# retinal-information-processing-lab/gaussian_processes

Hardware: AMD Instinct MI355X
Metric: GP fits/sec (kernel+chol+solve+grad loglik) at N=8192 d=256 (higher is better)
Workload: dtype f64; 1 GPU; N=8192 d=256 single cell f64, one M-step closure evaluation with 6 gradients (BASELINE configs[2], headline); N=8192, d=256, parallelism=independent units over 1 GPU(s), one process per GPU, no data-path collective

## Files before the change

gaussian_processes_amd/_lib.py:

```python
from __future__ import annotations

import ctypes
import os

from .build import lib_path

vp, i32, i64, f64 = ctypes.c_void_p, ctypes.c_int, ctypes.c_int64, ctypes.c_double
pd = ctypes.POINTER(ctypes.c_double)

_SIGS = {
    "gpfit_version": (i32, []),
    "gpfit_last_error": (ctypes.c_char_p, []),
    "gpfit_dgemm": (i32, [vp, i32, i32, i32, i32, i32, f64, vp, i64, vp, i64, f64, vp, i64, i32, i32, i32]),
    "gpfit_dgemm_ex": (i32, [vp, i32, i32, i32, i32, i32, f64, vp, i64, vp, i64, f64, vp, i64, i32, i32, i32, i32, i32]),
    "gpfit_ctx_create": (i32, [i32, i64, i64, i64, ctypes.POINTER(vp)]),
    "gpfit_ctx_destroy": (None, [vp]),
    "gpfit_check_limits": (i32, [pd, pd, pd]),
    "gpfit_localker_mask": (i32, [pd, i32, i32, vp, ctypes.POINTER(i64)]),
    "gpfit_localker": (i32, [vp, vp, pd, i32, i32, vp, i64, vp, vp]),
    "gpfit_acosker": (i32, [vp, vp, f64, vp, i64, i64, vp, i64, i64, i64, vp, i64, vp, vp, i64, vp]),
    "gpfit_acosker_pullback": (i32, [vp, vp, f64, vp, i64, i64, vp, i64, i64, i64, vp, i64, vp, i64, vp, vp, i64, pd]),
    "gpfit_acosker_diag": (i32, [vp, vp, f64, vp, i64, i64, i64, vp, i64, vp, vp, vp]),
    "gpfit_fit_eval": (i32, [vp, vp, pd, pd, pd, i32, i32, vp, i64, i64, vp, vp, vp, i64, f64, f64, i32, pd,
                             vp, vp, vp]),
    "gpfit_potrf": (i32, [vp, vp, vp, i64, i64, vp, i64, vp, i64, pd, ctypes.POINTER(i32)]),
    "gpfit_potrf_append": (i32, [vp, vp, vp, i64, vp, i64, i64, vp, pd, ctypes.POINTER(i32)]),
    "gpfit_estep": (i32, [vp, vp, vp, i64, i64, vp, vp, vp, f64, vp, vp, i64]),
    "gpfit_estep_projected": (i32, [vp, vp, vp, i64, vp, i64, vp, i64, i64, i64, vp, vp, vp, f64, vp, vp, i64, vp, vp,
                                    vp]),
    "gpfit_fparam_eval": (i32, [vp, vp, vp, vp, vp, i64, f64, i32, f64, vp, pd]),
    "gpfit_fparam_lbfgs": (i32, [vp, vp, vp, vp, vp, i64, f64, i32, f64, i32, i32, f64, f64, f64, vp, pd]),
    "gpfit_fparam_lbfgs_host": (i32, [vp, vp, vp, i64, f64, i32, f64, i32, i32, f64, f64, f64, vp, pd]),
    "gpfit_set_profile": (i32, [vp, i32]),
    "gpfit_get_profile": (i32, [vp, pd]),
    "gpfit_get_phases": (i32, [vp, pd]),
    "gpfit_last_enqueue_ms": (f64, [vp]),
    "gpfit_fit_eval_f32": (i32, [vp, vp, pd, pd, pd, i32, i32, vp, i64, i64, vp, vp, vp, i64, f64, f64, i32, pd,
                                 vp, vp, vp]),
    "gpfit_fit_eval_finish": (i32, [vp, pd]),
    "gpfit_fit_eval_batch": (i32, [vp, i32, vp, pd, pd, pd, i32, i32, vp, i64, i64, vp, vp, vp, i64, pd, pd, i32, pd,
                                   ctypes.POINTER(i32)]),
    "gpfit_fit_eval_batch_f32": (i32, [vp, i32, vp, pd, pd, pd, i32, i32, vp, i64, i64, vp, vp, vp, i64, pd, pd, i32, pd,
                                       ctypes.POINTER(i32)]),
    "gpfit_fit_eval_projected": (i32, [vp, vp, pd, pd, pd, i32, i32, vp, i64, i64, vp, vp, i64, i64, vp, vp, i64, f64, f64, pd]),
    "gpfit_fit_eval_sparse": (i32, [vp, vp, pd, pd, pd, i32, i32, vp, i64, i64, vp, i64, i64, vp, vp, i64, i64, vp, vp, i64,
                                    f64, f64, pd]),
    "gpfit_grad_pullback": (i32, [vp, vp, pd, i32, i32, vp, i64, i64, vp, i64, vp, pd]),
    "gpfit_nd_utility": (i32, [vp, vp, vp, i64, vp, i32, vp]),
    "gpfit_probe_mfma_f64": (i32, [vp, vp, i32, i32]),
    "gpfit_probe_stream_copy": (i32, [vp, vp, vp, i64]),
}

_lib = None


class GpfitError(RuntimeError):
    pass


def exported_symbols():
    return sorted(_SIGS)


def load():
    global _lib
    if _lib is not None:
        return _lib
    path = lib_path()
    if not os.path.exists(path):
        raise GpfitError(
            f"{path} not found: build it with `python -m gaussian_processes_amd.build` "
            "(there is no CPU fallback for the GP fit path)")
    lib = ctypes.CDLL(path)
    for name, (res, args) in _SIGS.items():
        fn = getattr(lib, name)
        fn.restype = res
        fn.argtypes = args
    _lib = lib
    return lib


def last_error() -> str:
    return load().gpfit_last_error().decode(errors="replace")
# ... 11 lines not shown
```

gaussian_processes_amd/csrc/common.h:

```cpp
#pragma once
#include <hip/hip_runtime.h>
#include <stdint.h>
#include <stdio.h>
#include <string>

namespace gpfit {

constexpr double PI32 = 3.1415927410125732;

constexpr int TILE = 128;
constexpr int TRMV_ROWS = 128;
constexpr int KTILE = 16;

void set_error(const std::string& msg);

#define GP_HIP(expr)                                                                     \
  do {                                                                                   \
    hipError_t _e = (expr);                                                              \
    if (_e != hipSuccess) {                                                              \
      gpfit::set_error(std::string(#expr) + ": " + hipGetErrorString(_e));               \
      return -100;                                                                       \
    }                                                                                    \
  } while (0)

// ... 21 lines not shown
  int batch;
  int64_t sA, sB, sC;
  int split_k;
  int tile;
  int reverse;
  int workspace;
  void* sk_ws;
  int tile_limit;
  int half_occ;
  const int* sched;
  int sched_blocks;
  int epi;
  R* aux;
  double* sumsq;
  int nptr;
  const R* Ap[GEMM_MAXB];
  const R* Bp[GEMM_MAXB];
  R* Cp[GEMM_MAXB];
  R* auxp[GEMM_MAXB];
  double* sumsqp[GEMM_MAXB];
};
using GemmArgs = GemmArgsT<double>;

constexpr size_t SK_WS_BYTES = (size_t)2 * 512 * TILE * TILE * sizeof(double);

template <typename R> constexpr int ktile_of() { return 128 / (int)sizeof(R); }

template <typename R> int launch_gemm(const GemmArgsT<R>& a, hipStream_t s);
template <typename R> int gemm_pick_tile(const GemmArgsT<R>& a);
template <typename R> int launch_gemm_streamk(const GemmArgsT<R>& a, hipStream_t s);
template <typename R> int launch_gemm_plain(const GemmArgsT<R>& a, hipStream_t s);
template <typename R> bool gemm_pair_ok(const GemmArgsT<R>& a, const GemmArgsT<R>& b);
template <typename R> int launch_gemm_pair(const GemmArgsT<R>& a, const GemmArgsT<R>& b, hipStream_t s);
template <typename R> int launch_gemm_xcd(const GemmArgsT<R>& a, hipStream_t s);
template <typename R> bool gemm_epilogue_ok(const GemmArgsT<R>& a);
template <typename R> bool gemm_streamk_applies(const GemmArgsT<R>& a);
template <typename R> bool gemm_streamk_carries(const GemmArgsT<R>& a);
template <typename R> int gemm_sumsq_entries(const GemmArgsT<R>& a);
template <typename R> bool gemm_xcd_applies(const GemmArgsT<R>& a);

template <typename R>
struct GramArgsT {
  const R* XCt;
  const R* Xt;
  const R* q1;
  const R* q2;
  R* Kout;
  R* Cos;
  int64_t ld1, ld2, ldk;
  int64_t ldcos;
  int np1, np2, nv1, nv2, Kd;
  double s0sq;
  int lower;
  int pad_identity;
  int mirror;
};
using GramArgs = GramArgsT<double>;
template <typename R> int launch_gram(const GramArgsT<R>& a, hipStream_t s);

}
```

gaussian_processes_amd/csrc/fit.hip:

```cpp
#include "context.h"
#include "gpfit_mi355x.h"

#include <algorithm>
#include <chrono>
#include <cmath>
#include <cstdlib>
#include <cstring>
#include <limits>

namespace gpfit {

static thread_local gpfit_ctx* g_prof = nullptr;
static thread_local void* g_main_sk_ws = nullptr;

static const int* walks() {
  static int w[7] = {3, 2, 1, 9, 9, 2, 2};
  static bool init = false;
  if (!init) {
    init = true;
    if (const char* e = getenv("GPFIT_WALKS")) {
      int v[7];
      if (sscanf(e, "%d,%d,%d,%d,%d,%d,%d", &v[0], &v[1], &v[2], &v[3], &v[4], &v[5], &v[6]) == 7)
        for (int i = 0; i < 7; ++i) w[i] = v[i];
    }
// ... 81 lines not shown
                              int b_tri, int reverse = 0, int ws = 0, void* sk_ws = nullptr) {
  GemmArgsT<R> g{};
  g.A = A; g.B = B; g.C = C;
  g.lda = lda; g.ldb = ldb; g.ldc = ldc;
  g.M = M; g.N = N; g.K = K;
  g.alpha = alpha; g.beta = beta;
  g.a_kmajor = a_kmajor; g.b_kmajor = b_kmajor;
  g.out_lower = out_lower; g.a_tri = a_tri; g.b_tri = b_tri;
  g.batch = 1; g.split_k = 1; g.reverse = reverse; g.workspace = ws; g.sk_ws = sk_ws ? sk_ws : g_main_sk_ws;
  return g;
}

static int g_eval_count = 0;
static int gemm_log_eval() {
  static const int v = getenv("GPFIT_GEMM_LOG") ? atoi(getenv("GPFIT_GEMM_LOG")) : -1;
  return v;
}

template <typename R>
static int run_gemm(hipStream_t s, const GemmArgsT<R>& g) {
  if (gemm_log_eval() >= 0 && g_eval_count == gemm_log_eval())
    fprintf(stderr, "[gpfit gemm] M %d N %d K %d atri %d btri %d lower %d nb %d tile %d ak %d bk %d epi %d flops %.6e\n", g.M, g.N, g.K,
            g.a_tri, g.b_tri, g.out_lower, g.nptr > 0 ? g.nptr : 1, gemm_pick_tile(g), g.a_kmajor, g.b_kmajor, g.epi, gemm_flops(g));
  ProfScope ps(s, g_prof ? gemm_flops(g) : 0.0, (g_prof && gemm_pick_tile(g) != TILE) ? 3 : 0);
  return launch_gemm(g, s);
}

template <typename R>
static int gemm(hipStream_t s, int a_kmajor, int b_kmajor, int M, int N, int K, double alpha, const R* A,
                int64_t lda, const R* B, int64_t ldb, double beta, R* C, int64_t ldc, int out_lower, int a_tri,
                int b_tri, int reverse = 0, int ws = 0, void* sk_ws = nullptr) {
  return run_gemm(s, gemm_args<R>(a_kmajor, b_kmajor, M, N, K, alpha, A, lda, B, ldb, beta, C, ldc, out_lower, a_tri, b_tri,
                                  reverse, ws, sk_ws));
}

template <typename R>
static int gemm_splitk(hipStream_t s, int a_kmajor, int b_kmajor, int M, int N, int K, double alpha, const R* A, int64_t lda,
                       const R* B, int64_t ldb, R* C, int64_t ldc, int splits, R* partial, int64_t partial_elems) {
  static const bool off = getenv("GPFIT_NO_SPLITK") != nullptr;
  splits = (int)std::min<int64_t>(splits, partial_elems / std::max<int64_t>(1, (int64_t)M * ldc));
  if (splits <= 1 || off || partial == nullptr)
    return gemm<R>(s, a_kmajor, b_kmajor, M, N, K, alpha, A, lda, B, ldb, 0.0, C, ldc, 0, 0, 0);
  GemmArgsT<R> g = gemm_args<R>(a_kmajor, b_kmajor, M, N, K, alpha, A, lda, B, ldb, 0.0, partial, ldc, 0, 0, 0);
  g.split_k = splits;
  g.sC = (int64_t)M * ldc;
  g.tile = TILE;
  GP_TRY(run_gemm(s, g));
  return launch_reduce_slices(partial, (int64_t)M * ldc, splits, C, (int64_t)M * ldc, s);
}
static int splitk_for(int M, int N, int K) {
  const long tiles = (long)((M + TILE - 1) / TILE) * ((N + TILE - 1) / TILE);
  if (tiles >= 384) return 1;
  long sp = (768 + tiles - 1) / tiles;
  sp = std::min<long>(sp, std::max(1, K / 256));
  return (int)std::max<long>(1, sp);
}

static int fused_epilogues() {
  static const int v = getenv("GPFIT_FUSED_EPI") ? atoi(getenv("GPFIT_FUSED_EPI")) : 7;
  return v;
}


template <typename R>
static int gemm_list(hipStream_t s, int cnt, const R* const* Ap, const R* const* Bp, R* const* Cp, int a_kmajor,
                     int b_kmajor, int M, int N, int K, double alpha, int64_t lda, int64_t ldb, double beta, int64_t ldc,
// ... 580 lines not shown
  const int kt = np / TILE, n1 = ((kt + 1) / 2) * TILE, n2 = np - n1;
  int ent = 0;
  auto asks = [&](int M, int Nn, int K, int lower, int a_tri, int b_tri, int walk) {
    GemmArgsT<R> g1 = gemm_args<R>(0, 1, M, Nn, K, 1.0, a[0].Li, ld, a[0].LV, ld, 0.0, a[0].T, ld, lower, a_tri, b_tri, walk, 0, cs[0]->sk_ws[0]);
    g1.epi = 2; g1.sumsq = cs[0]->frob_part;
    return ((fused_epilogues() & 2) && gemm_pick_tile(g1) == TILE) ? gemm_sumsq_entries(g1) : 0;
  };
  const bool any_fused = asks(n1, n1, n1, 1, 1, 1, walks()[3]) > 0 || asks(n2, n2, n2, 1, 1, 1, walks()[3]) > 0 ||
                         asks(n2, n1, n2, 0, 1, 0, walks()[2]) > 0;
  auto diag_blocks = [&](int cb, const int* rb, int nblk) -> int {
    const int tb = nblk / TILE;
    int e = asks(nblk, nblk, nblk, 1, 1, 1, walks()[3]);
    const bool ask = e > 0;
    if (!ask) e = tb * (tb + 1) / 2;
    int m = 0;
    for (int i = 0; i < cnt; ++i)
      for (int j = 0; j < cb; ++j, ++m) {
        const int64_t o = (int64_t)rb[j] * ld + rb[j];
        Ap[m] = a[i].Li + o; Bp[m] = a[i].LV + o; Tp[m] = a[i].T + o; Sp[m] = cs[i]->frob_part + ent + j * e;
      }
    bool normed = false;
    GP_TRY(gemm_list<R>(s, m, Ap, Bp, Tp, 0, 1, nblk, nblk, nblk, 1.0, ld, ld, 0.0, ld, 1, 1, 1, walks()[3], 0, cs[0]->sk_ws[0],
                        ask ? 2 : 0, nullptr, Sp, &normed));
    if (normed != ask) {
      set_error("post_join: the tile-norm epilogue of a diagonal block of T was announced but not carried");
      return -100;
    }
    if (!normed && any_fused)
      for (int q = 0; q < m; ++q) GP_TRY(launch_frob_tiles<R>(Tp[q], ld, nblk, nblk, 1, Sp[q], s));
    ent += cb * e;
    return 0;
  };
  const int r_both[2] = {0, n1};
  if (n2 == n1 && 2 * cnt <= GEMM_MAXB) GP_TRY(diag_blocks(2, r_both, n1));
  else {
    GP_TRY(diag_blocks(1, r_both, n1));
    GP_TRY(diag_blocks(1, r_both + 1, n2));
  }
  {
    const int64_t o21 = (int64_t)n1 * ld;
    for (int i = 0; i < cnt; ++i) {
      GP_HIP(hipMemcpy2DAsync(a[i].Z + o21, (size_t)ld * sizeof(R), a[i].LV + o21, (size_t)ld * sizeof(R), (size_t)n1 * sizeof(R),
                              (size_t)n2, hipMemcpyDeviceToDevice, s));
      Ap[i] = a[i].L + o21; Bp[i] = a[i].T; Cp[i] = a[i].Z + o21;
    }
    GP_TRY(gemm_list<R>(s, cnt, Ap, Bp, Cp, 0, 1, n2, n1, n1, -1.0, ld, ld, 1.0, ld, 0, 0, 1, walks()[1], 0, cs[0]->sk_ws[0]));
    int e = asks(n2, n1, n2, 0, 1, 0, walks()[2]);
    const bool ask = e > 0;
    if (!ask) e = (n2 / TILE) * (n1 / TILE);
    for (int i = 0; i < cnt; ++i) {
      Ap[i] = a[i].Li + o21 + n1; Bp[i] = a[i].Z + o21; Tp[i] = a[i].T + o21; Sp[i] = cs[i]->frob_part + ent;
    }
    bool normed = false;
    GP_TRY(gemm_list<R>(s, cnt, Ap, Bp, Tp, 0, 1, n2, n1, n2, 1.0, ld, ld, 0.0, ld, 0, 1, 0, walks()[2], 0, cs[0]->sk_ws[0],
                        ask ? 2 : 0, nullptr, Sp, &normed));
    if (normed != ask) {
      set_error("post_join: the tile-norm epilogue of T21 was announced but not carried");
      return -100;
    }
    if (!normed && any_fused)
      for (int i = 0; i < cnt; ++i) GP_TRY(launch_frob_tiles<R>(Tp[i], ld, n2, n1, 0, Sp[i], s));
    ent += e;
  }
  for (int i = 0; i < cnt; ++i) {
    if (any_fused) GP_TRY(launch_frob_finish(cs[i]->frob_part, ent, cs[i]->scal + 5, s));
    else GP_TRY(launch_frob_lower(a[i].T, ld, np, cs[i]->scal + 5, cs[i]->frob_part, s));
  }
  return 0;
}

template <typename R, typename PhaseFn>
static int post_join_list(int cnt, gpfit_ctx* const* cs, const PostJoin<R>* a, const Theta* th, int n, int np, const int* d,
                          const int* dp, int n_rows, int n_cols, int want_grad, bool blocks, hipStream_t s, PhaseFn&& phase) {
  const int64_t ld = np;
  const R* Ap[GEMM_MAXB];
  const R* Bp[GEMM_MAXB];
  R* Cp[GEMM_MAXB];
  double* Sp[GEMM_MAXB];
  if (cnt <= 0 || cnt > GEMM_MAXB) return cnt == 0 ? 0 : -3;
// ... 766 lines not shown
```

gaussian_processes_amd/csrc/gemm.hip:

```cpp
#include "gemm_core.h"

#include <algorithm>
#include <cstdlib>
#include <mutex>
#include <set>
#include <utility>

namespace gpfit {

template <typename R, bool A_KMAJOR, bool B_KMAJOR, bool EDGE, int T, int NS>
__device__ __forceinline__ bool gemm_tile_compute(const GemmArgsT<R>& p, int tiles_n, int ntiles, R* smem,
                                                  typename Real<R>::acc_t (&acc)[T / 32][T / 32], int& ti, int& tj,
                                                  int& row0, int& col0, R*& C) {
  constexpr int KT = Real<R>::KT;

  const int bid = (p.reverse & 1) ? (ntiles - 1 - (int)blockIdx.x) : (int)blockIdx.x;
  if (p.sched != nullptr) {
    const int e = p.sched[blockIdx.x];
    if (e < 0) return false;
    ti = e >> 16;
    tj = e & 0xffff;
  } else if (p.out_lower && (p.reverse & 2) && T == TILE) {
    const int nt = tiles_n;
    int j = (int)((2.0 * nt + 1.0 - sqrt((2.0 * nt + 1.0) * (2.0 * nt + 1.0) - 8.0 * (double)bid)) * 0.5);
    while (j > 0 && (long)j * nt - (long)j * (j - 1) / 2 > bid) --j;
    while ((long)(j + 1) * nt - (long)(j + 1) * j / 2 <= bid) ++j;
    tj = j;
    ti = j + (bid - (j * nt - j * (j - 1) / 2));
  } else if (p.out_lower) {
    lower_tile(bid, TILE / T, ti, tj);
  } else if (p.reverse & 2) {
    const int tiles_m = ntiles / tiles_n;
    tj = bid / tiles_m;
    ti = bid % tiles_m;
  } else {
    ti = bid / tiles_n;
    tj = bid % tiles_n;
  }
  row0 = ti * T;
  col0 = tj * T;
  const int b = blockIdx.y, z = blockIdx.z;
  const R* A;
  const R* B;
  if (p.nptr > 0) {
    A = p.Ap[b];
    B = p.Bp[b];
    C = p.Cp[b];
  } else {
    A = p.A + (int64_t)b * p.sA;
    B = p.B + (int64_t)b * p.sB;
    C = p.C + (int64_t)b * p.sC;
  }

  int kbeg = 0, kend = p.K;
  if (p.a_tri == 1) kend = min(kend, row0 + T);
  if (p.a_tri == 2) kbeg = max(kbeg, row0);
  if (p.b_tri == 1) kbeg = max(kbeg, col0);
  if (p.b_tri == 2) kend = min(kend, col0 + T);
  if (p.split_k > 1) {
    const int steps = max(0, kend - kbeg) / KT;
    const int per = (steps + p.split_k - 1) / p.split_k;
    const int s0 = min(steps, z * per), s1 = min(steps, (z + 1) * per);
    kend = kbeg + s1 * KT;
    kbeg = kbeg + s0 * KT;
    C += (int64_t)z * p.sC;
  }

#pragma unroll
  for (int i = 0; i < T / 32; ++i)
#pragma unroll
    for (int j = 0; j < T / 32; ++j) acc[i][j] = acc_zero<R>();

  gemm_mainloop<R, A_KMAJOR, B_KMAJOR, EDGE, T, 0, NS>(A, p.lda, B, p.ldb, p.M, p.N, row0, col0, kbeg, kend, smem, acc,
                                                       (p.reverse & 4) != 0);
  return true;
}

template <typename R, bool A_KMAJOR, bool B_KMAJOR, bool EDGE, int T, int NS, int EPI = 0>
__device__ __forceinline__ void gemm_tile_body(const GemmArgsT<R>& p, int tiles_n, int ntiles, R* smem) {
  typename Real<R>::acc_t acc[T / 32][T / 32];
  int ti, tj, row0, col0;
  R* C;
  if (!gemm_tile_compute<R, A_KMAJOR, B_KMAJOR, EDGE, T, NS>(p, tiles_n, ntiles, smem, acc, ti, tj, row0, col0, C)) return;

  const R alpha = (R)p.alpha, beta = (p.split_k > 1) ? (R)0 : (R)p.beta;
  const int64_t ldc = p.ldc;
  const int M = p.M, N = p.N;
  if constexpr (EPI != 0) {
    constexpr int epi = EPI;
    R* __restrict__ D = p.nptr > 0 ? p.auxp[blockIdx.y] : p.aux;
    double* __restrict__ sumsq = p.nptr > 0 ? p.sumsqp[blockIdx.y] : p.sumsq;
    double ss = 0.0;
    for_each_acc<R, T>(acc, row0, col0, [&](int row, int col, R v) {
      if (EDGE && !(row < M && col < N)) return;
      R o = alpha * v;
      R* c = C + (int64_t)row * ldc + col;
      if (epi & 4) {
        R* dd = D + (int64_t)row * ldc + col;
        const R d0 = *dd;
        o += d0;
        *dd = o + d0;
      } else if (beta != (R)0) {
        o += beta * (*c);
      }
      if (epi & 1) {
        if (row >= col) *c = o;
        if (row > col) C[(int64_t)col * ldc + row] = o;
// ... 274 lines not shown
int launch_gemm_pair(const GemmArgsT<R>& a, const GemmArgsT<R>& b, hipStream_t s) {
  if (!gemm_pair_ok(a, b)) {
    set_error("launch_gemm_pair: the two problems cannot share a launch (ask gemm_pair_ok first)");
    return -3;
  }
  static_assert(sizeof(GemmPairT<R>) <= 4096, "kernel arguments are limited to 4 KiB");
  const int T = pair_member_tile(a);
  GemmPairT<R> q;
  int gx = 0, gy = 0;
  long total = 0;
  for (int w = 0; w < 2; ++w) {
    q.g[w] = w == 0 ? a : b;
    GemmArgsT<R>& p = q.g[w];
    p.batch = p.nptr;
    const int tm = p.M / T, tn = p.N / T;
    q.tiles_n[w] = tn;
    q.tiles[w] = p.out_lower ? lower_tile_count(p.M / TILE, TILE / T) : tm * tn;
    gx = std::max(gx, q.tiles[w]);
    gy = std::max(gy, p.batch);
    total += (long)q.tiles[w] * p.batch;
  }
  const dim3 grid(gx, gy, 2), block(GEMM_THREADS);
  static const int deep_max = getenv("GPFIT_DEEP_MAX") ? atoi(getenv("GPFIT_DEEP_MAX")) : 512;
  if (T == 32 && total <= deep_max) hipLaunchKernelGGL((gemm_pair_kernel<R, 32, 8>), grid, block, 0, s, q);
  else if (T == 32) hipLaunchKernelGGL((gemm_pair_kernel<R, 32, 2>), grid, block, 0, s, q);
  else if (total <= deep_max) hipLaunchKernelGGL((gemm_pair_kernel<R, 64, 4>), grid, block, 0, s, q);
  else hipLaunchKernelGGL((gemm_pair_kernel<R, 64, 2>), grid, block, 0, s, q);
  GP_HIP(hipGetLastError());
  return 0;
}
template int launch_gemm_pair<double>(const GemmArgsT<double>&, const GemmArgsT<double>&, hipStream_t);
template int launch_gemm_pair<float>(const GemmArgsT<float>&, const GemmArgsT<float>&, hipStream_t);

template int launch_gemm<double>(const GemmArgsT<double>&, hipStream_t);
template int launch_gemm<float>(const GemmArgsT<float>&, hipStream_t);
template int launch_gemm_plain<double>(const GemmArgsT<double>&, hipStream_t);
template int launch_gemm_plain<float>(const GemmArgsT<float>&, hipStream_t);
template int gemm_pick_tile<double>(const GemmArgsT<double>&);
template int gemm_pick_tile<float>(const GemmArgsT<float>&);

}

#ifdef GPFIT_CLOCK_STAMPS
extern "C" int gpfit_dev_gemm_clock(long long* host_out ) {
  return hipMemcpyFromSymbol(host_out, HIP_SYMBOL(gpfit::g_gemm_clock), sizeof(long long) * 2 * 4096 * 2) == hipSuccess ? 0 : -1;
}
#endif
```

gaussian_processes_amd/csrc/gemm_sched.hip:

```cpp
#include "gemm_core.h"

#include <algorithm>
#include <cstdlib>
#include <map>
#include <mutex>
#include <tuple>
#include <vector>

namespace gpfit {

namespace {
struct Plan {
  int* table = nullptr;
  int blocks = 0;
};
using Key = std::tuple<int, int, int, int, int, int, int, int>;
std::map<Key, Plan> g_plans;
std::mutex g_mutex;

struct Item {
  long weight;
  std::vector<int> tiles;
};
}
// ... 76 lines not shown
}
template bool gemm_xcd_applies<double>(const GemmArgsT<double>&);
template bool gemm_xcd_applies<float>(const GemmArgsT<float>&);

template <typename R>
int launch_gemm_xcd(const GemmArgsT<R>& a, hipStream_t s) {
  if (!gemm_xcd_applies(a)) return 1;
  int device = 0;
  GP_HIP(hipGetDevice(&device));
  Plan plan;
  {
    std::lock_guard<std::mutex> lock(g_mutex);
    const Key key{device, a.M, a.N, a.K, a.out_lower, a.a_tri, a.b_tri, (int)sizeof(R)};
    auto it = g_plans.find(key);
    if (it == g_plans.end()) {
      Plan np;
      const int rc = build(a, np);
      if (rc != 0) return rc;
      it = g_plans.emplace(key, np).first;
    }
    plan = it->second;
  }
  GemmArgsT<R> p = a;
  p.tile = TILE;
  p.sched = plan.table;
  p.sched_blocks = plan.blocks;
  p.reverse &= 4;
  return launch_gemm_plain(p, s);
}

template int launch_gemm_xcd<double>(const GemmArgsT<double>&, hipStream_t);
template int launch_gemm_xcd<float>(const GemmArgsT<float>&, hipStream_t);

}
```

gaussian_processes_amd/csrc/probe.hip:

```cpp
#include "common.h"
#include "gpfit_mi355x.h"

namespace gpfit {
typedef double v4d __attribute__((ext_vector_type(4)));

#define GP_MFMA(acc) asm volatile("v_mfma_f64_16x16x4_f64 %0, %1, %2, %0" : "+v"(acc) : "v"(a), "v"(b))
__global__ __launch_bounds__(256) void mfma_f64_probe_kernel(double* out, int iters, double seed) {
  v4d c0 = {0, 0, 0, 0}, c1 = c0, c2 = c0, c3 = c0, c4 = c0, c5 = c0, c6 = c0, c7 = c0;
  v4d c8 = c0, c9 = c0, c10 = c0, c11 = c0, c12 = c0, c13 = c0, c14 = c0, c15 = c0;
  double a = seed + threadIdx.x * 1e-3, b = seed - threadIdx.x * 1e-3;
  for (int it = 0; it < iters; ++it) {
    GP_MFMA(c0); GP_MFMA(c1); GP_MFMA(c2); GP_MFMA(c3); GP_MFMA(c4); GP_MFMA(c5); GP_MFMA(c6); GP_MFMA(c7);
    GP_MFMA(c8); GP_MFMA(c9); GP_MFMA(c10); GP_MFMA(c11); GP_MFMA(c12); GP_MFMA(c13); GP_MFMA(c14); GP_MFMA(c15);
  }
  v4d s = c0 + c1 + c2 + c3 + c4 + c5 + c6 + c7 + c8 + c9 + c10 + c11 + c12 + c13 + c14 + c15;
  out[blockIdx.x * blockDim.x + threadIdx.x] = s[0] + s[1] + s[2] + s[3];
}
#undef GP_MFMA

__global__ void stream_copy_kernel(const double2* __restrict__ in, double2* __restrict__ out, int64_t n) {
  int64_t i = (int64_t)blockIdx.x * blockDim.x + threadIdx.x;
  const int64_t stride = (int64_t)gridDim.x * blockDim.x;
  for (; i < n; i += stride) out[i] = in[i];
}
}

extern "C" {

int gpfit_probe_mfma_f64(void* stream, double* scratch , int blocks, int iters) {
  hipLaunchKernelGGL(gpfit::mfma_f64_probe_kernel, dim3(blocks), dim3(256), 0, (hipStream_t)stream, scratch,
                     iters, 1.0);
  GP_HIP(hipGetLastError());
  return 0;
}

int gpfit_probe_stream_copy(void* stream, const double* in, double* out, int64_t n_doubles) {
  hipLaunchKernelGGL(gpfit::stream_copy_kernel, dim3(2048), dim3(256), 0, (hipStream_t)stream,
                     (const double2*)in, (double2*)out, n_doubles / 2);
  GP_HIP(hipGetLastError());
  return 0;
}
}
```

include/gpfit_mi355x.h:

```cpp
#ifndef GPFIT_MI355X_H
#define GPFIT_MI355X_H

#include <stdint.h>

#ifdef __cplusplus
extern "C" {
#endif

#define GPFIT_VERSION 100

int gpfit_version(void);
const char* gpfit_last_error(void);

int gpfit_dgemm(void* stream, int a_kmajor, int b_kmajor, int M, int N, int K, double alpha,
                const double* A, int64_t lda, const double* B, int64_t ldb, double beta, double* C,
                int64_t ldc, int out_lower, int a_tri, int b_tri);
int gpfit_dgemm_ex(void* stream, int a_kmajor, int b_kmajor, int M, int N, int K, double alpha,
                   const double* A, int64_t lda, const double* B, int64_t ldb, double beta, double* C,
                   int64_t ldc, int out_lower, int a_tri, int b_tri, int walk, int tile);

typedef struct gpfit_ctx gpfit_ctx;
int gpfit_ctx_create(int device, int64_t n_max, int64_t d_max, int64_t d_full_max, gpfit_ctx** out);
void gpfit_ctx_destroy(gpfit_ctx* ctx);

// ... 64 lines not shown
                          const double* L, int64_t ldl, int64_t N, int64_t nb, const double* r, const double* m,
                          const double* f, double logA, double* m_new, double* V_new, int64_t ldv, const double* kv0,
                          double* lam_m_out, double* lam_var_out);

int gpfit_fparam_eval(gpfit_ctx* ctx, void* stream, const double* lam_m, const double* lam_var,
                      const double* r, int64_t N, double logA, int closed_form_lambda0, double lambda0_in,
                      double* f_out, double* out_host);

int gpfit_fparam_lbfgs(gpfit_ctx* ctx, void* stream, const double* lam_m, const double* lam_var,
                       const double* r, int64_t N, double logA0, int lambda0_mode, double lambda0_fixed,
                       int max_iter, int history_size, double lr, double tol_grad, double tol_change,
                       double* f_out, double* out_host);
int gpfit_fparam_lbfgs_host(const double* lam_m, const double* lam_var, const double* r, int64_t N,
                            double logA0, int lambda0_mode, double lambda0_fixed, int max_iter,
                            int history_size, double lr, double tol_grad, double tol_change, double* f_out,
                            double* out_host);

int gpfit_nd_utility(void* stream, const double* sigma2, const double* mu, int64_t nstar, const double* r,
                     int nr, double* U);

int gpfit_set_profile(gpfit_ctx* ctx, int on);
int gpfit_get_profile(gpfit_ctx* ctx, double* out16);
int gpfit_get_phases(gpfit_ctx* ctx, double* out8);
double gpfit_last_enqueue_ms(gpfit_ctx* ctx);

int gpfit_fit_eval_f32(gpfit_ctx* ctx, void* stream, const double* theta, const double* lower,
                       const double* upper, int n_rows, int n_cols, const float* X, int64_t ldx, int64_t N,
                       const float* r, const float* m, const float* V, int64_t ldv, double logA, double lambda0,
                       int want_grad, double* out_host, float* lam_m, float* lam_var, float* f);

int gpfit_probe_mfma_f64(void* stream, double* scratch, int blocks, int iters);
int gpfit_probe_stream_copy(void* stream, const double* in, double* out, int64_t n_doubles);

#ifdef __cplusplus
}
#endif
#endif
```

Measured before the change: 35.92 fits/s.

## Fuse two dependent-free block GEMMs into one multi-problem launch with tile table

Adds a grouped GEMM kernel that runs several independent problems (up to 4 shapes × 16 members) in one launch, driven by a precomputed, load-balanced tile table cached on the device. In the blocked post-join step it merges the off-diagonal update (Z21 = LV21 - L21·T) with the lower-triangular 22 block product into one launch. It reads LV through an aux pointer in the epilogue, which removes the separate 2D device copy. This is meant to cut launch count, copy traffic and tail idle time. The cost is extra code paths, a fixed tile choice with no split-k or stream-k, and a plan cache held per shape.

```diff
diff --git a/gaussian_processes_amd/_lib.py b/gaussian_processes_amd/_lib.py
--- a/gaussian_processes_amd/_lib.py
+++ b/gaussian_processes_amd/_lib.py
@@ -49,6 +49,8 @@
     "gpfit_nd_utility": (i32, [vp, vp, vp, i64, vp, i32, vp]),
     "gpfit_probe_mfma_f64": (i32, [vp, vp, i32, i32]),
     "gpfit_probe_stream_copy": (i32, [vp, vp, vp, i64]),
+    "gpfit_probe_gemm_multi": (i32, [vp, i32, i32, i32, vp, vp, vp, vp]),
+    "gpfit_gemm_multi_table": (i32, [i32, vp, i32, i32, i32, vp, i32]),
 }
 
 _lib = None
diff --git a/gaussian_processes_amd/csrc/common.h b/gaussian_processes_amd/csrc/common.h
--- a/gaussian_processes_amd/csrc/common.h
+++ b/gaussian_processes_amd/csrc/common.h
@@ -77,6 +77,14 @@
 template <typename R> int launch_gemm_plain(const GemmArgsT<R>& a, hipStream_t s);
 template <typename R> bool gemm_pair_ok(const GemmArgsT<R>& a, const GemmArgsT<R>& b);
 template <typename R> int launch_gemm_pair(const GemmArgsT<R>& a, const GemmArgsT<R>& b, hipStream_t s);
+constexpr int MULTI_MAXD = 4;
+constexpr int MULTI_MAXB = 16;
+template <typename R> bool gemm_multi_ok(int nd, const GemmArgsT<R>* g);
+template <typename R> int gemm_multi_tile(int nd, const GemmArgsT<R>* g);
+template <typename R> int launch_gemm_multi(int nd, const GemmArgsT<R>* g, hipStream_t s);
+struct MultiShape { int M, N, K, out_lower, a_tri, b_tri; };
+int gemm_multi_table(int nd, const MultiShape* sh, int members, int T, int kstep, int* out, int cap);
+int gemm_multi_plan(int nd, const MultiShape* sh, int members, int T, int kstep, const int** table, int* blocks);
 template <typename R> int launch_gemm_xcd(const GemmArgsT<R>& a, hipStream_t s);
 template <typename R> bool gemm_epilogue_ok(const GemmArgsT<R>& a);
 template <typename R> bool gemm_streamk_applies(const GemmArgsT<R>& a);
diff --git a/gaussian_processes_amd/csrc/fit.hip b/gaussian_processes_amd/csrc/fit.hip
--- a/gaussian_processes_amd/csrc/fit.hip
+++ b/gaussian_processes_amd/csrc/fit.hip
@@ -137,6 +137,33 @@
                 int b_tri, int reverse = 0, int ws = 0, void* sk_ws = nullptr) {
   return run_gemm(s, gemm_args<R>(a_kmajor, b_kmajor, M, N, K, alpha, A, lda, B, ldb, beta, C, ldc, out_lower, a_tri, b_tri,
                                   reverse, ws, sk_ws));
+}
+
+static int no_multi() {
+  static const int v = getenv("GPFIT_NO_MULTI") ? atoi(getenv("GPFIT_NO_MULTI")) : 0;
+  return v;
+}
+
+template <typename R>
+static int run_gemm_multi(hipStream_t s, int nd, const GemmArgsT<R>* g) {
+  const int T = gemm_multi_tile(nd, g);
+  double flops = 0.0;
+  const bool log = gemm_log_eval() >= 0 && g_eval_count == gemm_log_eval();
+  if (log || g_prof)
+    for (int w = 0; w < nd; ++w) {
+      GemmArgsT<R> c = g[w];
+      c.tile = T;
+      flops += gemm_flops(c);
+    }
+  if (log) {
+    fprintf(stderr, "[gpfit gemm] multi: nd %d nb %d tile %d flops %.6e :", nd, g[0].nptr, T, flops);
+    for (int w = 0; w < nd; ++w)
+      fprintf(stderr, " [M %d N %d K %d atri %d btri %d lower %d epi %d]", g[w].M, g[w].N, g[w].K, g[w].a_tri, g[w].b_tri,
+              g[w].out_lower, g[w].epi);
+    fprintf(stderr, "\n");
+  }
+  ProfScope ps(s, g_prof ? flops : 0.0, (g_prof && T != TILE) ? 3 : 0);
+  return launch_gemm_multi(nd, g, s);
 }
 
 template <typename R>
@@ -783,19 +810,49 @@
     return 0;
   };
   const int r_both[2] = {0, n1};
-  if (n2 == n1 && 2 * cnt <= GEMM_MAXB) GP_TRY(diag_blocks(2, r_both, n1));
+  const int64_t o21 = (int64_t)n1 * ld, o22 = o21 + n1;
+  GemmArgsT<R> gm[2];
+  auto pair_args = [&](int i0, int m, bool ask22) {
+    gm[0] = gemm_args<R>(0, 1, n2, n1, n1, -1.0, (const R*)nullptr, ld, (const R*)nullptr, ld, 1.0, (R*)nullptr, ld, 0, 0, 1, walks()[1], 0,
+                         cs[0]->sk_ws[0]);
+    gm[1] = gemm_args<R>(0, 1, n2, n2, n2, 1.0, (const R*)nullptr, ld, (const R*)nullptr, ld, 0.0, (R*)nullptr, ld, 1, 1, 1, walks()[3], 0,
+                         cs[0]->sk_ws[0]);
+    gm[0].reverse &= 4; gm[1].reverse &= 4;
+    gm[1].epi = ask22 ? 2 : 0;
+    for (int w = 0; w < 2; ++w) { gm[w].nptr = m; gm[w].batch = m; }
+    for (int j = 0; j < m; ++j) {
+      const PostJoin<R>& u = a[i0 + j];
+      gm[0].Ap[j] = u.L + o21; gm[0].Bp[j] = u.T; gm[0].Cp[j] = u.Z + o21; gm[0].auxp[j] = const_cast<R*>(u.LV) + o21;
+      gm[1].Ap[j] = u.Li + o22; gm[1].Bp[j] = u.LV + o22; gm[1].Cp[j] = u.T + o22;
+      gm[1].sumsqp[j] = cs[i0 + j]->frob_part + ent;
+    }
+  };
+  const bool ask22 = asks(n2, n2, n2, 1, 1, 1, walks()[3]) > 0;
+  pair_args(0, std::min(cnt, MULTI_MAXB), ask22);
+  const bool multi = !(no_multi() & 1) && n2 > 0 && gemm_multi_ok(2, gm);
+  if (multi) {
+    GP_TRY(diag_blocks(1, r_both, n1));
+    for (int i0 = 0; i0 < cnt; i0 += MULTI_MAXB) {
+      pair_args(i0, std::min(cnt - i0, MULTI_MAXB), ask22);
+      GP_TRY(run_gemm_multi<R>(s, 2, gm));
+    }
+    if (!ask22 && any_fused)
+      for (int i = 0; i < cnt; ++i) GP_TRY(launch_frob_tiles<R>(a[i].T + o22, ld, n2, n2, 1, cs[i]->frob_part + ent, s));
+    ent += (n2 / TILE) * (n2 / TILE + 1) / 2;
+  } else if (n2 == n1 && 2 * cnt <= GEMM_MAXB) GP_TRY(diag_blocks(2, r_both, n1));
   else {
     GP_TRY(diag_blocks(1, r_both, n1));
     GP_TRY(diag_blocks(1, r_both + 1, n2));
   }
   {
-    const int64_t o21 = (int64_t)n1 * ld;
-    for (int i = 0; i < cnt; ++i) {
-      GP_HIP(hipMemcpy2DAsync(a[i].Z + o21, (size_t)ld * sizeof(R), a[i].LV + o21, (size_t)ld * sizeof(R), (size_t)n1 * sizeof(R),
-                              (size_t)n2, hipMemcpyDeviceToDevice, s));
-      Ap[i] = a[i].L + o21; Bp[i] = a[i].T; Cp[i] = a[i].Z + o21;
-    }
-    GP_TRY(gemm_list<R>(s, cnt, Ap, Bp, Cp, 0, 1, n2, n1, n1, -1.0, ld, ld, 1.0, ld, 0, 0, 1, walks()[1], 0, cs[0]->sk_ws[0]));
+    if (!multi) {
+      for (int i = 0; i < cnt; ++i) {
+        GP_HIP(hipMemcpy2DAsync(a[i].Z + o21, (size_t)ld * sizeof(R), a[i].LV + o21, (size_t)ld * sizeof(R), (size_t)n1 * sizeof(R),
+                                (size_t)n2, hipMemcpyDeviceToDevice, s));
+        Ap[i] = a[i].L + o21; Bp[i] = a[i].T; Cp[i] = a[i].Z + o21;
+      }
+      GP_TRY(gemm_list<R>(s, cnt, Ap, Bp, Cp, 0, 1, n2, n1, n1, -1.0, ld, ld, 1.0, ld, 0, 0, 1, walks()[1], 0, cs[0]->sk_ws[0]));
+    }
     int e = asks(n2, n1, n2, 0, 1, 0, walks()[2]);
     const bool ask = e > 0;
     if (!ask) e = (n2 / TILE) * (n1 / TILE);
diff --git a/gaussian_processes_amd/csrc/gemm.hip b/gaussian_processes_amd/csrc/gemm.hip
--- a/gaussian_processes_amd/csrc/gemm.hip
+++ b/gaussian_processes_amd/csrc/gemm.hip
@@ -7,6 +7,17 @@
 #include <utility>
 
 namespace gpfit {
+
+template <typename R, bool A_KMAJOR, bool B_KMAJOR, bool EDGE, int T, int NS>
+__device__ __forceinline__ void gemm_tile_product(const R* A, int64_t lda, const R* B, int64_t ldb, int M, int N, int row0,
+                                                  int col0, int kbeg, int kend, R* smem,
+                                                  typename Real<R>::acc_t (&acc)[T / 32][T / 32], bool kdesc) {
+#pragma unroll
+  for (int i = 0; i < T / 32; ++i)
+#pragma unroll
+    for (int j = 0; j < T / 32; ++j) acc[i][j] = acc_zero<R>();
+  gemm_mainloop<R, A_KMAJOR, B_KMAJOR, EDGE, T, 0, NS>(A, lda, B, ldb, M, N, row0, col0, kbeg, kend, smem, acc, kdesc);
+}
 
 template <typename R, bool A_KMAJOR, bool B_KMAJOR, bool EDGE, int T, int NS>
 __device__ __forceinline__ bool gemm_tile_compute(const GemmArgsT<R>& p, int tiles_n, int ntiles, R* smem,
@@ -66,13 +77,8 @@
     C += (int64_t)z * p.sC;
   }
 
-#pragma unroll
-  for (int i = 0; i < T / 32; ++i)
-#pragma unroll
-    for (int j = 0; j < T / 32; ++j) acc[i][j] = acc_zero<R>();
-
-  gemm_mainloop<R, A_KMAJOR, B_KMAJOR, EDGE, T, 0, NS>(A, p.lda, B, p.ldb, p.M, p.N, row0, col0, kbeg, kend, smem, acc,
-                                                       (p.reverse & 4) != 0);
+  gemm_tile_product<R, A_KMAJOR, B_KMAJOR, EDGE, T, NS>(A, p.lda, B, p.ldb, p.M, p.N, row0, col0, kbeg, kend, smem, acc,
+                                                        (p.reverse & 4) != 0);
   return true;
 }
 
@@ -413,6 +419,157 @@
 template int launch_gemm_pair<double>(const GemmArgsT<double>&, const GemmArgsT<double>&, hipStream_t);
 template int launch_gemm_pair<float>(const GemmArgsT<float>&, const GemmArgsT<float>&, hipStream_t);
 
+template <typename R>
+struct GemmDescT {
+  int64_t lda, ldb, ldc;
+  int M, N, K;
+  double alpha, beta;
+  int out_lower, a_tri, b_tri, epi, tiles_n, kdesc;
+  const R* Ap[MULTI_MAXB];
+  const R* Bp[MULTI_MAXB];
+  R* Cp[MULTI_MAXB];
+  R* auxp[MULTI_MAXB];
+  double* sumsqp[MULTI_MAXB];
+};
+template <typename R>
+struct GemmMultiT {
+  GemmDescT<R> d[MULTI_MAXD];
+  const int* table;
+};
+
+template <typename R, int T, int NS>
+__device__ __forceinline__ void gemm_multi_body(const GemmMultiT<R>& q, R* smem) {
+  const int e = q.table[blockIdx.x];
+  if (e < 0) return;
+  const int w = e >> 29, b = (e >> 24) & 31, ti = (e >> 12) & 0xfff, tj = e & 0xfff;
+  const GemmDescT<R>& d = q.d[w];
+  const int row0 = ti * T, col0 = tj * T;
+  int kbeg = 0, kend = d.K;
+  if (d.a_tri == 1) kend = min(kend, row0 + T);
+  if (d.a_tri == 2) kbeg = max(kbeg, row0);
+  if (d.b_tri == 1) kbeg = max(kbeg, col0);
+  if (d.b_tri == 2) kend = min(kend, col0 + T);
+  typename Real<R>::acc_t acc[T / 32][T / 32];
+  gemm_tile_product<R, false, true, false, T, NS>(d.Ap[b], d.lda, d.Bp[b], d.ldb, d.M, d.N, row0, col0, kbeg, kend, smem, acc,
+                                                  d.kdesc != 0);
+  R* __restrict__ C = d.Cp[b];
+  const R alpha = (R)d.alpha, beta = (R)d.beta;
+  const int64_t ldc = d.ldc;
+  if (T == TILE && d.epi == 2) {
+    double ss = 0.0;
+    for_each_acc<R, T>(acc, row0, col0, [&](int row, int col, R v) {
+      R o = alpha * v;
+      R* c = C + (int64_t)row * ldc + col;
+      if (beta != (R)0) o += beta * (*c);
+      *c = o;
+      ss += (double)o * (double)o;
+    });
+#pragma unroll
+    for (int o = 32; o > 0; o >>= 1) ss += __shfl_down(ss, o);
+    double* red = reinterpret_cast<double*>(smem);
+    __syncthreads();
+    if ((threadIdx.x & 63) == 0) red[threadIdx.x >> 6] = ss;
+    __syncthreads();
+    if (threadIdx.x == 0)
+      d.sumsqp[b][d.out_lower ? (int64_t)ti * (ti + 1) / 2 + tj : (int64_t)ti * d.tiles_n + tj] = (red[0] + red[1]) + (red[2] + red[3]);
+    return;
+  }
+  if (beta == (R)0) {
+    for_each_acc<R, T>(acc, row0, col0, [&](int row, int col, R v) { C[(int64_t)row * ldc + col] = alpha * v; });
+  } else {
+    const R* __restrict__ src = d.auxp[b] != nullptr ? d.auxp[b] : C;
+    for_each_acc<R, T>(acc, row0, col0, [&](int row, int col, R v) {
+      const int64_t o = (int64_t)row * ldc + col;
+      C[o] = alpha * v + beta * src[o];
+    });
+  }
+}
+
+template <typename R, int T, int NS>
+__global__ __launch_bounds__(GEMM_THREADS, (T == 128 || NS > 2 ? 2 : 4)) void gemm_multi_kernel(GemmMultiT<R> q) {
+  __shared__ __attribute__((aligned(16))) R smem[2 * NS * Real<R>::KT * T];
+  gemm_multi_body<R, T, NS>(q, smem);
+}
+
+template <typename R>
+static void multi_shapes(int nd, const GemmArgsT<R>* g, MultiShape* sh) {
+  for (int w = 0; w < nd; ++w) sh[w] = MultiShape{g[w].M, g[w].N, g[w].K, g[w].out_lower, g[w].a_tri, g[w].b_tri};
+}
+
+template <typename R>
+int gemm_multi_tile(int nd, const GemmArgsT<R>* g) {
+  static const long t128_min = getenv("GPFIT_MULTI_T128_MIN") ? atol(getenv("GPFIT_MULTI_T128_MIN")) : 512;
+  long tiles = 0;
+  for (int w = 0; w < nd; ++w) {
+    const long tm = g[w].M / TILE, tn = g[w].N / TILE;
+    tiles += (g[w].out_lower ? tm * (tm + 1) / 2 : tm * tn) * std::max(1, g[w].nptr);
+  }
+  return tiles >= t128_min ? TILE : 64;
+}
+
+template <typename R>
+bool gemm_multi_ok(int nd, const GemmArgsT<R>* g) {
+  constexpr int EPC = 16 / (int)sizeof(R);
+  if (nd < 1 || nd > MULTI_MAXD) return false;
+  for (int w = 0; w < nd; ++w) {
+    const GemmArgsT<R>& a = g[w];
+    if (a.nptr < 1 || a.nptr > MULTI_MAXB || a.nptr != g[0].nptr) return false;
+    if (a.a_kmajor || !a.b_kmajor || a.split_k > 1 || a.sched || a.half_occ || a.tile_limit || a.tile) return false;
+    if (a.M <= 0 || a.N <= 0 || a.K <= 0 || (a.M % TILE) || (a.N % TILE) || (a.out_lower && a.M != a.N)) return false;
+    if (a.M / 64 >= 4096 || a.N / 64 >= 4096) return false;
+    if (a.K % ktile_of<R>() != 0 || (a.lda % EPC) || (a.ldb % EPC)) return false;
+    if (a.epi != 0 && a.epi != 2) return false;
+    for (int b = 0; b < a.nptr; ++b)
+      if (a.epi == 2 && a.sumsqp[b] == nullptr) return false;
+  }
+  if (gemm_multi_tile(nd, g) != TILE)
+    for (int w = 0; w < nd; ++w)
+      if (g[w].epi == 2) return false;
+  return true;
+}
+
+template <typename R>
+int launch_gemm_multi(int nd, const GemmArgsT<R>* g, hipStream_t s) {
+  if (!gemm_multi_ok(nd, g)) {
+    set_error("launch_gemm_multi: these problems cannot share a launch (ask gemm_multi_ok first)");
+    return -3;
+  }
+  static_assert(sizeof(GemmMultiT<R>) <= 4096, "kernel arguments are limited to 4 KiB");
+  const int T = gemm_multi_tile(nd, g);
+  GemmMultiT<R> q{};
+  MultiShape sh[MULTI_MAXD];
+  multi_shapes(nd, g, sh);
+  for (int w = 0; w < nd; ++w) {
+    const GemmArgsT<R>& a = g[w];
+    GemmDescT<R>& d = q.d[w];
+    d.lda = a.lda; d.ldb = a.ldb; d.ldc = a.ldc;
+    d.M = a.M; d.N = a.N; d.K = a.K;
+    d.alpha = a.alpha; d.beta = a.beta;
+    d.out_lower = a.out_lower; d.a_tri = a.a_tri; d.b_tri = a.b_tri; d.epi = a.epi;
+    d.tiles_n = a.N / T;
+    d.kdesc = (a.reverse & 4) != 0;
+    for (int b = 0; b < a.nptr; ++b) {
+      d.Ap[b] = a.Ap[b]; d.Bp[b] = a.Bp[b]; d.Cp[b] = a.Cp[b];
+      d.auxp[b] = a.auxp[b]; d.sumsqp[b] = a.sumsqp[b];
+    }
+  }
+  int blocks = 0;
+  GP_TRY(gemm_multi_plan(nd, sh, g[0].nptr, T, ktile_of<R>(), &q.table, &blocks));
+  const dim3 grid(blocks), block(GEMM_THREADS);
+  static const int deep_max = getenv("GPFIT_DEEP_MAX") ? atoi(getenv("GPFIT_DEEP_MAX")) : 512;
+  if (T == TILE) hipLaunchKernelGGL((gemm_multi_kernel<R, TILE, 2>), grid, block, 0, s, q);
+  else if (blocks <= deep_max) hipLaunchKernelGGL((gemm_multi_kernel<R, 64, 4>), grid, block, 0, s, q);
+  else hipLaunchKernelGGL((gemm_multi_kernel<R, 64, 2>), grid, block, 0, s, q);
+  GP_HIP(hipGetLastError());
+  return 0;
+}
+template bool gemm_multi_ok<double>(int, const GemmArgsT<double>*);
+template bool gemm_multi_ok<float>(int, const GemmArgsT<float>*);
+template int gemm_multi_tile<double>(int, const GemmArgsT<double>*);
+template int gemm_multi_tile<float>(int, const GemmArgsT<float>*);
+template int launch_gemm_multi<double>(int, const GemmArgsT<double>*, hipStream_t);
+template int launch_gemm_multi<float>(int, const GemmArgsT<float>*, hipStream_t);
+
 template int launch_gemm<double>(const GemmArgsT<double>&, hipStream_t);
 template int launch_gemm<float>(const GemmArgsT<float>&, hipStream_t);
 template int launch_gemm_plain<double>(const GemmArgsT<double>&, hipStream_t);
diff --git a/gaussian_processes_amd/csrc/gemm_sched.hip b/gaussian_processes_amd/csrc/gemm_sched.hip
--- a/gaussian_processes_amd/csrc/gemm_sched.hip
+++ b/gaussian_processes_amd/csrc/gemm_sched.hip
@@ -132,4 +132,116 @@
 template int launch_gemm_xcd<double>(const GemmArgsT<double>&, hipStream_t);
 template int launch_gemm_xcd<float>(const GemmArgsT<float>&, hipStream_t);
 
-}
+namespace {
+struct MultiItem {
+  long weight;
+  std::vector<int> tiles;
+};
+using MultiKey = std::vector<int>;
+std::map<MultiKey, Plan> g_multi_plans;
+}
+
+static std::vector<int> multi_table(int nd, const MultiShape* sh, int members, int T, int kstep) {
+  static const long min_tiles = getenv("GPFIT_XCD_MIN_TILES") ? atol(getenv("GPFIT_XCD_MIN_TILES")) : 1536;
+  const int r = TILE / T;
+  auto ksteps = [&](const MultiShape& p, int ti, int tj) {
+    int kb = 0, ke = p.K;
+    if (p.a_tri == 1) ke = std::min(ke, ti * T + T);
+    if (p.a_tri == 2) kb = std::max(kb, ti * T);
+    if (p.b_tri == 1) kb = std::max(kb, tj * T);
+    if (p.b_tri == 2) ke = std::min(ke, tj * T + T);
+    return (long)std::max(0, ke - kb) / kstep;
+  };
+  long total_tiles = 0;
+  for (int w = 0; w < nd; ++w) {
+    const long tm = sh[w].M / TILE, tn = sh[w].N / TILE;
+    total_tiles += sh[w].out_lower ? tm * (tm + 1) / 2 : tm * tn;
+  }
+  const bool deal = T == TILE && total_tiles >= min_tiles;
+  const int G = deal ? 2 : 1;
+  std::vector<MultiItem> items;
+  for (int w = 0; w < nd; ++w) {
+    const int tm = sh[w].M / T, tn = sh[w].N / T;
+    for (int I = 0; I < tm; I += G)
+      for (int J = 0; J < tn; J += G) {
+        MultiItem it;
+        it.weight = 0;
+        for (int ti = I; ti < std::min(I + G, tm); ++ti)
+          for (int tj = J; tj < std::min(J + G, tn); ++tj) {
+            if (sh[w].out_lower && tj / r > ti / r) continue;
+            it.tiles.push_back((w << 29) | (ti << 12) | tj);
+            it.weight += ksteps(sh[w], ti, tj);
+          }
+        if (!it.tiles.empty()) items.push_back(std::move(it));
+      }
+  }
+  std::stable_sort(items.begin(), items.end(), [](const MultiItem& x, const MultiItem& y) { return x.weight > y.weight; });
+  std::vector<int> one;
+  if (deal) {
+    std::vector<int> queue[8];
+    long load[8] = {0, 0, 0, 0, 0, 0, 0, 0};
+    for (auto& it : items) {
+      int best = 0;
+      for (int x = 1; x < 8; ++x)
+        if (load[x] < load[best]) best = x;
+      load[best] += it.weight;
+      queue[best].insert(queue[best].end(), it.tiles.begin(), it.tiles.end());
+    }
+    size_t len = 0;
+    for (auto& q : queue) len = std::max(len, q.size());
+    one.assign(8 * len, -1);
+    for (int x = 0; x < 8; ++x)
+      for (size_t i = 0; i < queue[x].size(); ++i) one[8 * i + x] = queue[x][i];
+  } else {
+    for (auto& it : items) one.insert(one.end(), it.tiles.begin(), it.tiles.end());
+  }
+  std::vector<int> table;
+  table.reserve(one.size() * members);
+  for (int b = 0; b < members; ++b)
+    for (int e : one) table.push_back(e < 0 ? -1 : (e | (b << 24)));
+  return table;
+}
+
+static bool multi_shapes_ok(int nd, const MultiShape* sh, int members, int T, int kstep) {
+  if (nd < 1 || nd > MULTI_MAXD || members < 1 || members > MULTI_MAXB || (T != TILE && T != 64) || kstep <= 0) return false;
+  for (int w = 0; w < nd; ++w) {
+    const MultiShape& p = sh[w];
+    if (p.M <= 0 || p.N <= 0 || p.K <= 0 || (p.M % TILE) || (p.N % TILE) || (p.K % kstep)) return false;
+    if (p.M / T >= 4096 || p.N / T >= 4096 || (p.out_lower && p.M != p.N)) return false;
+  }
+  return true;
+}
+
+int gemm_multi_table(int nd, const MultiShape* sh, int members, int T, int kstep, int* out, int cap) {
+  if (!multi_shapes_ok(nd, sh, members, T, kstep)) return -3;
+  const std::vector<int> table = multi_table(nd, sh, members, T, kstep);
+  if (out != nullptr)
+    for (size_t i = 0; i < table.size() && (int)i < cap; ++i) out[i] = table[i];
+  return (int)table.size();
+}
+
+int gemm_multi_plan(int nd, const MultiShape* sh, int members, int T, int kstep, const int** table, int* blocks) {
+  if (!multi_shapes_ok(nd, sh, members, T, kstep)) {
+    set_error("gemm_multi_plan: shapes a multi launch cannot take");
+    return -3;
+  }
+  int device = 0;
+  GP_HIP(hipGetDevice(&device));
+  MultiKey key{device, members, T, kstep};
+  for (int w = 0; w < nd; ++w) key.insert(key.end(), {sh[w].M, sh[w].N, sh[w].K, sh[w].out_lower, sh[w].a_tri, sh[w].b_tri});
+  std::lock_guard<std::mutex> lock(g_mutex);
+  auto it = g_multi_plans.find(key);
+  if (it == g_multi_plans.end()) {
+    const std::vector<int> host = multi_table(nd, sh, members, T, kstep);
+    Plan np;
+    np.blocks = (int)host.size();
+    GP_HIP(hipMalloc((void**)&np.table, host.size() * sizeof(int)));
+    GP_HIP(hipMemcpy(np.table, host.data(), host.size() * sizeof(int), hipMemcpyHostToDevice));
+    it = g_multi_plans.emplace(key, np).first;
+  }
+  *table = it->second.table;
+  *blocks = it->second.blocks;
+  return 0;
+}
+
+}
diff --git a/gaussian_processes_amd/csrc/probe.hip b/gaussian_processes_amd/csrc/probe.hip
--- a/gaussian_processes_amd/csrc/probe.hip
+++ b/gaussian_processes_amd/csrc/probe.hip
@@ -40,4 +40,56 @@
   GP_HIP(hipGetLastError());
   return 0;
 }
+
+int gpfit_probe_gemm_multi(void* stream, int nd, int members, int separate, const int* shape, const double* coef,
+                           const int64_t* ld, const void* const* ptrs) {
+  using namespace gpfit;
+  hipStream_t s = (hipStream_t)stream;
+  if (nd < 1 || nd > MULTI_MAXD || members < 1 || members > MULTI_MAXB) {
+    set_error("gpfit_probe_gemm_multi: 1..4 problems of 1..16 members");
+    return -3;
+  }
+  GemmArgsT<double> g[MULTI_MAXD];
+  for (int w = 0; w < nd; ++w) {
+    GemmArgsT<double>& a = g[w];
+    a = GemmArgsT<double>{};
+    const int* sh = shape + 7 * w;
+    a.M = sh[0]; a.N = sh[1]; a.K = sh[2]; a.out_lower = sh[3]; a.a_tri = sh[4]; a.b_tri = sh[5]; a.epi = sh[6];
+    a.alpha = coef[2 * w]; a.beta = coef[2 * w + 1];
+    a.lda = ld[3 * w]; a.ldb = ld[3 * w + 1]; a.ldc = ld[3 * w + 2];
+    a.a_kmajor = 0; a.b_kmajor = 1; a.batch = 1; a.split_k = 1;
+    a.nptr = members;
+    for (int b = 0; b < members; ++b) {
+      const void* const* p = ptrs + ((size_t)w * members + b) * 5;
+      a.Ap[b] = (const double*)p[0]; a.Bp[b] = (const double*)p[1]; a.Cp[b] = (double*)p[2];
+      a.auxp[b] = (double*)p[3]; a.sumsqp[b] = (double*)p[4];
+    }
+  }
+  if (!separate) return launch_gemm_multi(nd, g, s);
+  for (int w = 0; w < nd; ++w)
+    for (int b = 0; b < members; ++b) {
+      GemmArgsT<double> a = g[w];
+      a.nptr = 0;
+      a.A = g[w].Ap[b]; a.B = g[w].Bp[b]; a.C = g[w].Cp[b]; a.aux = nullptr; a.sumsq = g[w].sumsqp[b];
+      if (a.epi == 2) a.tile = TILE;
+      if (a.epi == 0 && g[w].auxp[b] != nullptr)
+        GP_HIP(hipMemcpy2DAsync(a.C, (size_t)a.ldc * sizeof(double), g[w].auxp[b], (size_t)a.ldc * sizeof(double),
+                                (size_t)a.N * sizeof(double), (size_t)a.M, hipMemcpyDeviceToDevice, s));
+      if (a.epi && !gemm_epilogue_ok(a)) {
+        set_error("gpfit_probe_gemm_multi: the separate launch cannot carry the epilogue");
+        return -3;
+      }
+      GP_TRY(launch_gemm_plain(a, s));
+    }
+  return 0;
 }
+
+int gpfit_gemm_multi_table(int nd, const int* shape, int members, int tile, int kstep, int* out, int cap) {
+  using namespace gpfit;
+  if (nd < 1 || nd > MULTI_MAXD || shape == nullptr) return -3;
+  MultiShape sh[MULTI_MAXD];
+  for (int w = 0; w < nd; ++w)
+    sh[w] = MultiShape{shape[6 * w], shape[6 * w + 1], shape[6 * w + 2], shape[6 * w + 3], shape[6 * w + 4], shape[6 * w + 5]};
+  return gemm_multi_table(nd, sh, members, tile, kstep, out, cap);
+}
+}
diff --git a/include/gpfit_mi355x.h b/include/gpfit_mi355x.h
--- a/include/gpfit_mi355x.h
+++ b/include/gpfit_mi355x.h
@@ -120,6 +120,10 @@
 int gpfit_probe_mfma_f64(void* stream, double* scratch, int blocks, int iters);
 int gpfit_probe_stream_copy(void* stream, const double* in, double* out, int64_t n_doubles);
 
+int gpfit_probe_gemm_multi(void* stream, int nd, int members, int separate, const int* shape, const double* coef,
+                           const int64_t* ld, const void* const* ptrs);
+int gpfit_gemm_multi_table(int nd, const int* shape, int members, int tile, int kstep, int* out, int cap);
+
 #ifdef __cplusplus
 }
 #endif
```

Measured after the change: 36.12 fits/s, median of 5. About the same (+0.6%).
